# DIG-Beihang/RobustART

Hardware: AMD Instinct MI355X
Metric: corrupted+attacked images/sec/node (ResNet-50, PGD-7 + IN-C x5) (higher is better)
Workload: dtype bf16x3; 1 GPU; per step and GPU: gaussian_noise sev 1..5 on 256 u8 224x224 images -> normalise -> ResNet-50 eval (1280 img) + PGD-Linf-7 eps 2/255 ResNet-50 eval (256 img); global_batch=256, parallelism=dp1, streams=2

## Files before the change

### include/robustart_hip.h

```cpp
#ifndef ROBUSTART_HIP_H
#define ROBUSTART_HIP_H

#include <stddef.h>
#include <stdint.h>

#ifdef __cplusplus
extern "C" {
#endif

typedef void* rart_stream_t;

typedef enum rart_status {
  RART_OK = 0,
  RART_ERR_INVALID = 1,
  RART_ERR_UNSUPPORTED = 2,
  RART_ERR_WORKSPACE = 3,
  RART_ERR_HIP = 4
} rart_status;

enum {
  RART_GAUSSIAN_NOISE = 0, RART_SHOT_NOISE = 1, RART_IMPULSE_NOISE = 2, RART_DEFOCUS_BLUR = 3,
  RART_GLASS_BLUR = 4, RART_MOTION_BLUR = 5, RART_ZOOM_BLUR = 6, RART_SNOW = 7, RART_FROST = 8,
  RART_FOG = 9, RART_BRIGHTNESS = 10, RART_CONTRAST = 11, RART_ELASTIC_TRANSFORM = 12,
  RART_PIXELATE = 13, RART_JPEG_COMPRESSION = 14, RART_SPECKLE_NOISE = 15, RART_GAUSSIAN_BLUR = 16,
// ... 186 lines not shown
typedef struct rart_gemm_pair_cls_desc {
  rart_gemm_pair2_desc two;
  int n_classes, reserved_;
  rart_gemm_pair_class cls[4];
} rart_gemm_pair_cls_desc;
int rart_gemm_pair_classes_bf16(const rart_gemm_pair_cls_desc* desc_host, rart_stream_t stream);
int rart_gemm_pair_max_classes(void);
int rart_gemm_pair_set_schedule(int mode);
int rart_gemm_pair_get_schedule(void);

typedef struct rart_conv_tail_desc {
  const void* a_hi;  const void* a_lo;
  const void* w_hi;  const void* w_lo;
  const void* t_hi;  const void* t_lo;
  const float* bias_mid;
  const float* bias_out;
  const void* mask_mid;  const void* mask_out;
  void* sign_mid;  void* sign_out;
  const void* res_hi;  const void* res_lo;
  void* dst_hi;  void* dst_lo;
  int batch, h, w, c_mid, ldw, relu_mid, relu_out;
  int tap_dy[9], tap_dx[9];
  const void* n_hi;  const void* n_lo;
  const float* bias_next;
  const void* mask_next;
  void* sign_next;
  void* dstn_hi;  void* dstn_lo;
  int relu_next;
  const void* x_hi;  const void* x_lo;
  const void* tx_hi;  const void* tx_lo;
} rart_conv_tail_desc;
int rart_conv3x3_tail_pair_supported(int c_mid);
int rart_conv3x3_tail_pair(const rart_conv_tail_desc* desc_host, rart_stream_t stream);

int rart_vit_add_pos_cls_pair(void* x_hi, void* x_lo, const float* cls_pos0, const float* pos, int n, int tokens, int dim,
                              rart_stream_t stream);
int rart_layernorm_pair(const void* x_hi, const void* x_lo, const float* gamma, const float* beta, void* out_hi, void* out_lo, int rows,
                        int dim, int64_t in_row_stride, int64_t out_row_stride, float eps, rart_stream_t stream);
int rart_layernorm_bwd_pair(const void* dy_hi, const void* dy_lo, const void* x_hi, const void* x_lo, const float* gamma,
                            const void* res_hi, const void* res_lo, void* dx_hi, void* dx_lo, int rows, int dim, int64_t dy_row_stride,
                            int64_t x_row_stride, int64_t res_row_stride, int64_t dx_row_stride, float eps, rart_stream_t stream);
int rart_softmax_rows_pair(const float* scores, void* probs_hi, void* probs_lo, int64_t rows, int n_valid, int ld_in, int ld_out,
                           float scale, rart_stream_t stream);
int rart_softmax_bwd_rows_pair(const void* probs_hi, const void* probs_lo, const float* dprobs, void* ds_hi, void* ds_lo, int64_t rows,
                               int n_valid, int ld_p, int ld_dp, int ld_out, float scale, rart_stream_t stream);
int rart_vit_unpatchify_from_f32(const float* dpatches, float* grad, int n, int h, int w, int patch, int64_t ld, const float* std_host,
                                 rart_stream_t stream);
int rart_vit_attention_pair(const void* qkv_hi, const void* qkv_lo, void* out_hi, void* out_lo, int n, int tokens, int heads, int head_dim,
                            rart_stream_t stream);
int rart_vit_attention_bwd_pair(const void* qkv_hi, const void* qkv_lo, const void* out_hi, const void* out_lo, const void* dout_hi,
                                const void* dout_lo, void* dqkv_hi, void* dqkv_lo, float* stats, int n, int tokens, int heads, int head_dim,
                                rart_stream_t stream);

int rart_conv3x3_halo_supported(int channels, int h, int w);
int rart_conv3x3_pack_frag_bf16(const void* w_rows, void* w_frag, int channels, rart_stream_t stream);
int rart_pack_frag_bf16(const void* w_rows, void* w_frag, int rows, int k, rart_stream_t stream);
int rart_conv3x3_halo_bf16(const void* src, const void* wgt, const float* bias, const void* mask_bits, void* sign_out,
                           void* dst, int n, int h, int w, int channels, const int* tap_dy, const int* tap_dx, int relu,
                           rart_stream_t stream);

int rart_bottleneck_fused_supported(int c_io, int c_mid, int h, int w);
int rart_bottleneck_fused_bf16(const void* x, const void* w1, const void* w2, const void* w3, const float* b1, const float* b2,
                               const float* b3, void* m1, void* m2, void* m3, void* out, int n, int h, int w, int c_io,
                               int c_mid, const int* tap_dy, const int* tap_dx, int backward, rart_stream_t stream);

int rart_bottleneck_first_supported(int c_in, int c_mid, int c_out, int h, int w);
// ... 306 lines not shown
```

### robustart_amd/_lib.py

```python
import ctypes
import os

_HERE = os.path.dirname(os.path.abspath(__file__))
LIB_PATH = os.path.join(_HERE, 'lib', 'librobustart_hip.so')

c_void_p, c_int, c_size_t, c_u64, c_float = (ctypes.c_void_p, ctypes.c_int, ctypes.c_size_t,
                                              ctypes.c_uint64, ctypes.c_float)
c_double = ctypes.c_double

ABI_VERSION = 110

SIGNATURES = {
    'rart_version': (c_int, []),
    'rart_last_error_string': (ctypes.c_char_p, []),
    'rart_corruption_name': (ctypes.c_char_p, [c_int]),
    'rart_corrupt_workspace_bytes': (c_size_t, [c_int, c_int, c_int, c_int, c_int]),
    'rart_corrupt_u8': (c_int, [c_void_p, c_void_p, c_int, c_int, c_int, c_int, c_int, c_u64, c_u64,
                                ctypes.POINTER(c_void_p), c_int, c_void_p, c_size_t, c_void_p]),
    'rart_stencil_fixed_point_info': (c_int, [c_int, c_int, c_void_p, c_void_p, c_size_t]),
    'rart_noise_multi_u8': (c_int, [c_void_p, ctypes.POINTER(c_void_p), c_int, c_int, c_int, c_int, c_int, ctypes.POINTER(c_int),
                                    ctypes.POINTER(c_u64), c_u64, c_void_p]),
    'rart_frost_textures_u8': (c_int, [c_void_p, c_void_p, c_int, c_int, c_int, c_int, c_void_p, c_int, c_int, c_int, ctypes.POINTER(c_int),
                                       c_u64, c_u64, c_void_p]),
    'rart_pil_resize_workspace_bytes': (c_size_t, [c_int] * 10),
# ... 77 lines not shown
    'rart_bottleneck_fused_bf16': (c_int, [c_void_p] * 11 + [c_int] * 5 + [ctypes.POINTER(c_int), ctypes.POINTER(c_int), c_int,
                                           c_void_p]),
    'rart_igemm_set_bk64_min_k': (c_int, [ctypes.c_longlong]),
    'rart_gemm_small_m_bf16': (c_int, [c_void_p, c_int, c_void_p, c_int, c_void_p, c_void_p, c_int, c_int, c_int, c_int, c_int, c_void_p]),
    'rart_igemm_set_gemm256': (c_int, [c_int]),
    'rart_gemm256_supported': (c_int, [ctypes.c_longlong, c_int, c_int, c_int, c_int]),
    'rart_gemm_pair_bf16': (c_int, [c_void_p, c_void_p]),
    'rart_copy_calibration': (c_int, [c_void_p, c_void_p, ctypes.c_size_t, c_int, c_void_p]),
    'rart_gemm_pair_set_schedule': (c_int, [c_int]),
    'rart_gemm_pair_get_schedule': (c_int, []),
    'rart_pack_jobs_bf16': (c_int, [c_void_p, c_int, c_int, c_void_p]),
    'rart_vit_add_pos_cls_pair': (c_int, [c_void_p, c_void_p, c_void_p, c_void_p, c_int, c_int, c_int, c_void_p]),
    'rart_layernorm_pair': (c_int, [c_void_p] * 6 + [c_int, c_int, ctypes.c_int64, ctypes.c_int64, c_float, c_void_p]),
    'rart_layernorm_bwd_pair': (c_int, [c_void_p] * 9 + [c_int, c_int] + [ctypes.c_int64] * 4 + [c_float, c_void_p]),
    'rart_softmax_rows_pair': (c_int, [c_void_p, c_void_p, c_void_p, ctypes.c_int64, c_int, c_int, c_int, c_float, c_void_p]),
    'rart_softmax_bwd_rows_pair': (c_int, [c_void_p] * 5 + [ctypes.c_int64, c_int, c_int, c_int, c_int, c_float, c_void_p]),
    'rart_vit_attention_pair': (c_int, [c_void_p, c_void_p, c_void_p, c_void_p, c_int, c_int, c_int, c_int, c_void_p]),
    'rart_vit_attention_bwd_pair': (c_int, [c_void_p] * 9 + [c_int, c_int, c_int, c_int, c_void_p]),
    'rart_vit_unpatchify_from_f32': (c_int, [c_void_p, c_void_p, c_int, c_int, c_int, c_int, ctypes.c_int64, ctypes.POINTER(c_float), c_void_p]),
    'rart_engine_prep_input': (c_int, [c_void_p, c_int, c_void_p, c_void_p, c_int, c_int, c_int, c_void_p, c_void_p,
                                       c_void_p]),
    'rart_engine_maxpool': (c_int, [c_void_p, c_void_p, c_void_p, c_int, c_int, c_int, c_int, c_void_p]),
    'rart_engine_maxpool_keep': (c_int, [c_void_p, c_void_p, c_void_p, c_void_p, c_int, c_int, c_int, c_int, c_void_p]),
    'rart_engine_maxpool_bwd': (c_int, [c_void_p, c_void_p, c_void_p, c_void_p, c_int, c_int, c_int, c_int, c_void_p]),
    'rart_engine_avgpool': (c_int, [c_void_p, c_void_p, c_int, c_int, c_int, c_void_p]),
    'rart_engine_avgpool_bwd': (c_int, [c_void_p, c_void_p, c_void_p, c_int, c_int, c_int, c_void_p]),
    'rart_engine_stem_col2im': (c_int, [c_void_p, c_void_p, c_int, c_int, c_int, c_int, c_void_p, c_void_p]),
    'rart_engine_stem_fwd_fused': (c_int, [c_void_p, c_int, c_void_p, c_int, c_void_p, c_void_p, c_void_p, c_void_p, c_int, c_int,
                                           c_int, c_void_p, c_void_p, c_void_p]),
    'rart_wgrad_direct_supported': (c_int, [c_int, c_int, c_int]),
    'rart_wgrad_direct_bf16': (c_int, [c_void_p, c_void_p, c_void_p] + [c_int] * 10 + [c_void_p, c_void_p, c_int, c_int, c_int, c_void_p]),
    'rart_conv3x3_tail_pair_supported': (c_int, [c_int]),
    'rart_conv3x3_tail_pair': (c_int, [c_void_p, c_void_p]),
    'rart_engine_stem_fwd_fused_pair': (c_int, [c_void_p, c_int] + [c_void_p] * 7 + [c_int, c_int, c_int, c_void_p, c_void_p, c_void_p]),
    'rart_engine_stem_fwd_next_pair': (c_int, [c_void_p, c_int] + [c_void_p] * 9 + [c_int] + [c_void_p] * 4 + [c_int, c_int, c_int, c_void_p, c_void_p,
                                               c_void_p]),
    'rart_engine_stem_bwd_fused_pair': (c_int, [c_void_p] * 6 + [c_int, c_int, c_int, c_void_p, c_void_p]),
    'rart_engine_stem_bwd_fused': (c_int, [c_void_p, c_void_p, c_void_p, c_void_p, c_int, c_int, c_int, c_void_p, c_void_p]),
    'rart_engine_maxpool_pair': (c_int, [c_void_p, ctypes.c_longlong, c_void_p, ctypes.c_longlong, c_void_p, c_void_p, c_int, c_int, c_int, c_int, c_void_p]),
    'rart_engine_maxpool_bwd_pair': (c_int, [c_void_p, c_void_p, ctypes.c_longlong, c_void_p, ctypes.c_longlong, c_int, c_int, c_int, c_int, c_void_p]),
    'rart_engine_avgpool_pair': (c_int, [c_void_p, ctypes.c_longlong, c_void_p, ctypes.c_longlong, c_int, c_int, c_int, c_void_p]),
    'rart_engine_avgpool_bwd_pair': (c_int, [c_void_p, c_void_p, ctypes.c_longlong, c_void_p, ctypes.c_longlong, c_int, c_int, c_int, c_void_p]),
    'rart_f32_to_pair_rows': (c_int, [c_void_p, c_void_p, ctypes.c_longlong, c_int, c_int, c_int, c_void_p]),
    'rart_engine_stem_col2im_f32': (c_int, [c_void_p, c_void_p, c_int, c_int, c_int, c_int, c_void_p, c_void_p]),
    'rart_f32_to_bf16_rows': (c_int, [c_void_p, c_void_p, c_int, c_int, c_int, c_void_p]),
    'rart_cnx_dwconv_ln_bf16': (c_int, [c_void_p] * 7 + [c_int] * 4 + [c_float, c_void_p]),
    'rart_cnx_dwconv_ln_pair': (c_int, [c_void_p] * 10 + [c_int] * 4 + [c_float, c_void_p]),
    'rart_cnx_dwconv_bwd_bf16': (c_int, [c_void_p] * 4 + [c_int] * 4 + [c_void_p]),
    'rart_cnx_dwconv_bwd_pair': (c_int, [c_void_p] * 7 + [c_int] * 4 + [c_void_p]),
    'rart_cnx_pool_bwd_bf16': (c_int, [c_void_p, c_void_p, c_int, c_int, c_int, c_void_p]),
    'rart_cnx_pool_bwd_pair': (c_int, [c_void_p] * 4 + [c_int, c_int, c_int, c_void_p]),
    'rart_cnx_patchify': (c_int, [c_void_p, c_int, c_void_p, c_void_p, c_int, c_int, c_int, c_int, c_int, c_void_p, c_void_p, c_void_p]),
    'rart_cvst_im2col': (c_int, [c_void_p, c_int, c_void_p, c_void_p, c_int, c_int, c_int, c_int, c_void_p, c_void_p, c_void_p]),
    'rart_cvst_col2im_f32': (c_int, [c_void_p, c_void_p, c_int, c_int, c_int, c_int, c_void_p, c_void_p]),
    'rart_ln_gelu_bf16': (c_int, [c_void_p] * 4 + [c_int, c_int, ctypes.c_int64, ctypes.c_int64, c_float, c_void_p]),
    'rart_ln_gelu_pair': (c_int, [c_void_p] * 6 + [c_int, c_int, ctypes.c_int64, ctypes.c_int64, c_float, c_void_p]),
    'rart_ln_gelu_bwd_bf16': (c_int, [c_void_p] * 5 + [c_int, c_int] + [ctypes.c_int64] * 3 + [c_float, c_void_p]),
    'rart_ln_gelu_bwd_pair': (c_int, [c_void_p] * 8 + [c_int, c_int] + [ctypes.c_int64] * 3 + [c_float, c_void_p]),
    'rart_cnx_dwconv_wgrad_workspace_bytes': (c_size_t, [c_int] * 4),
    'rart_cnx_dwconv_wgrad_bf16': (c_int, [c_void_p] * 4 + [c_int] * 6 + [c_void_p, c_size_t, c_void_p]),
    'rart_cnx_layer_scale_fwd_bf16': (c_int, [c_void_p] * 4 + [ctypes.c_longlong, c_int, c_void_p]),
    'rart_cnx_layer_scale_bwd_workspace_bytes': (c_size_t, [ctypes.c_longlong, c_int]),
    'rart_cnx_layer_scale_bwd_bf16': (c_int, [c_void_p] * 6 + [ctypes.c_longlong, c_int, c_int, c_void_p, c_size_t, c_void_p]),
    'rart_cnx_grn_stats_bf16': (c_int, [c_void_p] * 2 + [c_int] * 3 + [c_void_p]),
    'rart_cnx_grn_stats_pair': (c_int, [c_void_p] * 3 + [c_int] * 3 + [c_void_p]),
    'rart_cnx_grn_apply_bf16': (c_int, [c_void_p] * 5 + [c_int] * 3 + [c_float, c_void_p]),
# ... 260 lines not shown
```

### robustart_amd/csrc/conv_tail_pair.hip

```cpp
#include "rart_common.h"
#include "rart_lds_dma.h"

typedef __attribute__((ext_vector_type(8))) __bf16 bf16x8;
typedef __attribute__((ext_vector_type(16))) float f32x16;

namespace {
constexpr int CT_TM = 128;
constexpr int CT_LDE = 68;
constexpr int CT_PLANE_A = CT_TM * 64;
constexpr int CT_NLD = 144;
constexpr int CT_WREG = 2 * 32 * CT_NLD;
static_assert(CT_WREG >= 32 * CT_LDE * 4, "the staging must fit the wave's region");

struct ConvTailDev {
  const uint16_t *a_hi, *a_lo, *w_hi, *w_lo, *t_hi, *t_lo;
  const float *bias_mid, *bias_out;
  const uint8_t *mask_mid, *mask_out;
  uint8_t *sign_mid, *sign_out;
  const uint16_t *res_hi, *res_lo;
  uint16_t *dst_hi, *dst_lo;
  int M, H, W, ldw, relu_mid, relu_out;
  int tap_dy[9], tap_dx[9];
  uint32_t w_magic, w_shift, h_magic, h_shift;
  const uint16_t *n_hi, *n_lo;
  const float* bias_next;
  const uint8_t* mask_next;
  uint8_t* sign_next;
  uint16_t *dstn_hi, *dstn_lo;
  int relu_next;
  const uint16_t *x_hi, *x_lo, *tx_hi, *tx_lo;
};
typedef __attribute__((ext_vector_type(4))) uint32_t ct_u4;
__device__ __forceinline__ uint4 ct_nt_load(const uint16_t* p) {
  const ct_u4 v = __builtin_nontemporal_load(reinterpret_cast<const ct_u4*>(p));
  return make_uint4(v[0], v[1], v[2], v[3]);
}
__device__ __forceinline__ void ct_nt_store(uint16_t* p, const uint4& v) {
  ct_u4 w = {v.x, v.y, v.z, v.w};
  __builtin_nontemporal_store(w, reinterpret_cast<ct_u4*>(p));
}
__device__ __forceinline__ uint32_t ct_fastdiv(uint32_t n, uint32_t magic, uint32_t shift) { return (uint32_t)(((uint64_t)n * magic) >> shift); }

__device__ __forceinline__ uint32_t ct_pack_bf16x2(float lo, float hi) {
  typedef __attribute__((ext_vector_type(2))) float f2_t;
  typedef __attribute__((ext_vector_type(2))) __bf16 b2_t;
// ... 31 lines not shown

template <int NJ>
__device__ __forceinline__ void ct_pointwise_frags(const f32x16* acc, const uint32_t* mw, bool relu, int h, uint4* fh, uint4* fl) {
#pragma unroll
  for (int j = 0; j < NJ; ++j)
#pragma unroll
    for (int ge = 0; ge < 4; ge += 2) {
      uint32_t eh[2], el[2], oh[2], ol[2];
#pragma unroll
      for (int w = 0; w < 2; ++w) {
        float ve[2], vo[2];
#pragma unroll
        for (int i = 0; i < 2; ++i) {
          ve[i] = acc[j][4 * ge + 2 * w + i];
          vo[i] = acc[j][4 * ge + 4 + 2 * w + i];
          if (relu) { ve[i] = fmaxf(ve[i], 0.f); vo[i] = fmaxf(vo[i], 0.f); }
          if (!((mw[j] >> (8 * ge + 4 * h + 2 * w + i)) & 1u)) ve[i] = 0.f;
          if (!((mw[j] >> (8 * ge + 8 + 4 * h + 2 * w + i)) & 1u)) vo[i] = 0.f;
        }
        eh[w] = ct_pack_bf16x2(ve[0], ve[1]);
        el[w] = ct_pack_bf16x2(ve[0] - __uint_as_float(eh[w] << 16), ve[1] - __uint_as_float(eh[w] & 0xFFFF0000u));
        oh[w] = ct_pack_bf16x2(vo[0], vo[1]);
        ol[w] = ct_pack_bf16x2(vo[0] - __uint_as_float(oh[w] << 16), vo[1] - __uint_as_float(oh[w] & 0xFFFF0000u));
        const auto sh = __builtin_amdgcn_permlane32_swap(eh[w], oh[w], false, false);
        eh[w] = sh[0]; oh[w] = sh[1];
        const auto sl = __builtin_amdgcn_permlane32_swap(el[w], ol[w], false, false);
        el[w] = sl[0]; ol[w] = sl[1];
      }
      fh[j * 2 + ge / 2] = make_uint4(eh[0], eh[1], oh[0], oh[1]);
      fl[j * 2 + ge / 2] = make_uint4(el[0], el[1], ol[0], ol[1]);
    }
}

template <int C, bool NEXT, bool XS = false>
__global__ __launch_bounds__(256, (C == 64 && !NEXT && !XS) ? 3 : 2) void k_conv3x3_tail_pair(const ConvTailDev d) {
  static_assert(!XS || C == 64, "the shortcut source is built for layer1's first block: 64 input channels");
  constexpr int KX = 4;
  constexpr int NJ = C / 32;
  constexpr int KS = C / 16;
  constexpr int NOUT = 4 * C, NC = NOUT / 64;
  constexpr int TPT_SHIFT = C == 64 ? 1 : 2;
  constexpr int KT = 9 << TPT_SHIFT;
  constexpr int PLANE_B = C * 64, STAGE = 2 * CT_PLANE_A + 2 * PLANE_B;
  constexpr int BQ = (C / 16) / 4;
  static_assert(4 * CT_WREG <= 2 * STAGE, "the waves' epilogue regions must fit the tile buffers");
  __shared__ __attribute__((aligned(16))) uint8_t lds[2 * STAGE];
  const int tid = threadIdx.x, lane = tid & 63;
  const int wave = __builtin_amdgcn_readfirstlane(tid >> 6);
  uint32_t tile;
  {
    const uint32_t nb = gridDim.x, bid = blockIdx.x, xcd = bid & 7u, slot = bid >> 3, q = nb >> 3, r = nb & 7u;
    tile = (xcd < r ? xcd * (q + 1u) : r * (q + 1u) + (xcd - r) * q) + slot;
  }
  const int m0 = (int)tile * CT_TM;

  uint32_t avoff[2], nok[2] = {0u, 0u};
  int tap_min = 0;
  for (int t = 0; t < 9; ++t) tap_min = min(tap_min, (d.tap_dy[t] * d.W + d.tap_dx[t]) * (C * 2));
  const int tapreg = lane < 9 ? (d.tap_dy[lane] * d.W + d.tap_dx[lane]) * (C * 2) - tap_min : 0;
#pragma unroll
  for (int q = 0; q < 2; ++q) {
    const int r = 16 * (wave + 4 * q) + (lane >> 2);
    const int cs = ((lane & 3) ^ ((r >> 2) & 3)) * 16;
    const int m = m0 + r;
    const bool ok = m < d.M;
    const uint32_t mm = ok ? (uint32_t)m : 0u;
    const uint32_t t = ct_fastdiv(mm, d.w_magic, d.w_shift);
    const int ax = (int)(mm - t * (uint32_t)d.W);
    const int n = (int)ct_fastdiv(t, d.h_magic, d.h_shift);
    const int ay = (int)(t - (uint32_t)n * (uint32_t)d.H);
    avoff[q] = (uint32_t)((n * d.H * d.W + ay * d.W + ax) * (C * 2) + cs);
    for (int t2 = 0; t2 < 9; ++t2) {
      const int iy = ay + d.tap_dy[t2], ix = ax + d.tap_dx[t2];
      if (!(ok && (unsigned)iy < (unsigned)d.H && (unsigned)ix < (unsigned)d.W)) nok[q] |= 1u << t2;
    }
  }
  uint32_t wvoff[BQ];
#pragma unroll
  for (int q = 0; q < BQ; ++q) {
    const int r = 16 * (wave + 4 * q) + (lane >> 2);
    wvoff[q] = (uint32_t)((r * d.ldw + (((lane & 3) ^ ((r >> 2) & 3)) * 8)) * 2);
  }
  const rart_srd_t srd_ah = rart_dma_srd(reinterpret_cast<const char*>(d.a_hi) + tap_min), srd_al = rart_dma_srd(reinterpret_cast<const char*>(d.a_lo) + tap_min);
  const rart_srd_t srd_wh = rart_dma_srd(d.w_hi), srd_wl = rart_dma_srd(d.w_lo);
  const uint32_t lds_base = (uint32_t)(uintptr_t)(__attribute__((address_space(3))) uint8_t*)lds;
#define RART_CT_ISSUE(KT_, BUF)                                                                                 \
  {                                                                                                             \
    const uint32_t st_ = lds_base + (BUF)*STAGE;                                                                \
    const int kt_ = (KT_);                                                                                      \
    const int tap_ = kt_ >> TPT_SHIFT;                                                                          \
    const uint32_t so_ = (uint32_t)(__builtin_amdgcn_readlane(tapreg, tap_) + (kt_ - (tap_ << TPT_SHIFT)) * 64); \
    _Pragma("unroll") for (int q = 0; q < 2; ++q) {                                                             \
      const uint32_t vo_ = avoff[q] | ((uint32_t)__builtin_amdgcn_sbfe(nok[q], tap_, 1) & RART_DMA_OOR);        \
      rart_dma_load16(vo_, srd_ah, so_, st_ + (wave + 4 * q) * 1024);                                           \
      rart_dma_load16(vo_, srd_al, so_, st_ + CT_PLANE_A + (wave + 4 * q) * 1024);                              \
    }                                                                                                           \
    _Pragma("unroll") for (int q = 0; q < BQ; ++q) {                                                            \
      rart_dma_load16(wvoff[q], srd_wh, (uint32_t)kt_ * 64u, st_ + 2 * CT_PLANE_A + (wave + 4 * q) * 1024);     \
      rart_dma_load16(wvoff[q], srd_wl, (uint32_t)kt_ * 64u, st_ + 2 * CT_PLANE_A + PLANE_B + (wave + 4 * q) * 1024); \
    }                                                                                                           \
  }
  const int fr = lane & 31, h = lane >> 5;
  uint32_t xo[2];
#pragma unroll
  for (int ks = 0; ks < 2; ++ks) xo[ks] = (uint32_t)(fr * 64 + (((2 * ks + h) ^ ((fr >> 2) & 3)) << 4));
  f32x16 acc[NJ];
#pragma unroll
  for (int j = 0; j < NJ; ++j)
#pragma unroll
    for (int g = 0; g < 4; ++g) {
      float4 bv = make_float4(0.f, 0.f, 0.f, 0.f);
      if (d.bias_mid) bv = *reinterpret_cast<const float4*>(d.bias_mid + j * 32 + 8 * g + 4 * h);
      acc[j][4 * g] = bv.x; acc[j][4 * g + 1] = bv.y; acc[j][4 * g + 2] = bv.z; acc[j][4 * g + 3] = bv.w;
    }
  RART_CT_ISSUE(0, 0)
  rart_dma_wait<0>();
  __syncthreads();
  for (int kt = 0; kt < KT; ++kt) {
    const int buf = kt & 1;
    if (kt + 1 < KT) RART_CT_ISSUE(kt + 1, buf ^ 1)
    const uint8_t* Pb = lds + buf * STAGE + (wave * 32) * 64;
    const uint8_t* Wb = lds + buf * STAGE + 2 * CT_PLANE_A;
#pragma unroll
    for (int ks = 0; ks < 2; ++ks) {
      const bf16x8 ph = *reinterpret_cast<const bf16x8*>(Pb + xo[ks]);
      const bf16x8 pl = *reinterpret_cast<const bf16x8*>(Pb + CT_PLANE_A + xo[ks]);
#pragma unroll
      for (int j = 0; j < NJ; ++j) {
        const bf16x8 wh = *reinterpret_cast<const bf16x8*>(Wb + j * 32 * 64 + xo[ks]);
        const bf16x8 wl = *reinterpret_cast<const bf16x8*>(Wb + PLANE_B + j * 32 * 64 + xo[ks]);
        acc[j] = __builtin_amdgcn_mfma_f32_32x32x16_bf16(wh, pl, acc[j], 0, 0, 0);
        acc[j] = __builtin_amdgcn_mfma_f32_32x32x16_bf16(wl, ph, acc[j], 0, 0, 0);
        acc[j] = __builtin_amdgcn_mfma_f32_32x32x16_bf16(wh, ph, acc[j], 0, 0, 0);
      }
    }
    rart_dma_wait<0>();
    __syncthreads();
  }
#undef RART_CT_ISSUE

  const int p = m0 + wave * 32 + fr;
  const bool p_ok = p < d.M;
  bf16x8 a2h[KS], a2l[KS];
  {
    uint32_t mw[NJ];
#pragma unroll
    for (int j = 0; j < NJ; ++j) mw[j] = 0xFFFFFFFFu;
    if (d.mask_mid && p_ok) {
      const uint32_t* mp = reinterpret_cast<const uint32_t*>(d.mask_mid + (size_t)p * (C / 8));
#pragma unroll
      for (int j = 0; j < NJ; ++j) mw[j] = mp[j];
    }
    uint4 fh[KS], fl[KS];
    ct_pointwise_frags<NJ>(acc, mw, d.relu_mid != 0, h, fh, fl);
#pragma unroll
    for (int s = 0; s < KS; ++s) {
      a2h[s] = __builtin_bit_cast(bf16x8, fh[s]);
      a2l[s] = __builtin_bit_cast(bf16x8, fl[s]);
      if (d.sign_mid && p_ok) d.sign_mid[(size_t)p * (C / 8) + 2 * s + h] = (uint8_t)ct_sign_byte(fh[s]);
    }
  }

  bf16x8 xfh[XS ? KX : 1], xfl[XS ? KX : 1];
  if (XS) {
#pragma unroll
    for (int s = 0; s < KX; ++s) {
      uint4 vh = make_uint4(0, 0, 0, 0), vl = vh;
      if (p_ok) {
        vh = *reinterpret_cast<const uint4*>(d.x_hi + (size_t)p * 64 + 16 * s + 8 * h);
        vl = *reinterpret_cast<const uint4*>(d.x_lo + (size_t)p * 64 + 16 * s + 8 * h);
      }
      xfh[s] = __builtin_bit_cast(bf16x8, vh);
// ... 159 lines not shown
      }
      __builtin_amdgcn_fence(__ATOMIC_RELEASE, "wavefront");
      __builtin_amdgcn_wave_barrier();
    }
  }
  if (NEXT) {
    uint32_t mw[NJ];
#pragma unroll
    for (int j = 0; j < NJ; ++j) mw[j] = 0xFFFFFFFFu;
    if (d.mask_next && p_ok) {
      const uint32_t* mp = reinterpret_cast<const uint32_t*>(d.mask_next + (size_t)p * (C / 8));
#pragma unroll
      for (int j = 0; j < NJ; ++j) mw[j] = mp[j];
    }
    uint4 fh[KS], fl[KS];
    ct_pointwise_frags<NJ>(accn, mw, d.relu_next != 0, h, fh, fl);
    if (p_ok) {
#pragma unroll
      for (int s = 0; s < KS; ++s) {
        ct_nt_store(d.dstn_hi + (size_t)p * C + 16 * s + 8 * h, fh[s]);
        ct_nt_store(d.dstn_lo + (size_t)p * C + 16 * s + 8 * h, fl[s]);
        if (d.sign_next) d.sign_next[(size_t)p * (C / 8) + 2 * s + h] = (uint8_t)ct_sign_byte(fh[s]);
      }
    }
  }
}

void ct_magic(uint32_t dv, uint32_t& mg, uint32_t& sh) {
  uint32_t l = 0;
  while ((1ull << l) < dv) ++l;
  sh = 31 + l;
  mg = (uint32_t)(((1ull << sh) + dv - 1) / dv);
}
}

extern "C" int rart_conv3x3_tail_pair_supported(int c_mid) { return (c_mid == 64 || c_mid == 128) ? 1 : 0; }

extern "C" int rart_conv3x3_tail_pair(const rart_conv_tail_desc* t, rart_stream_t stream) {
  RART_CHECK_ARG(t != nullptr, "rart_conv3x3_tail_pair: null descriptor");
  RART_CHECK_ARG(t->a_hi && t->a_lo && t->w_hi && t->w_lo && t->t_hi && t->t_lo && t->dst_hi && t->dst_lo,
                 "rart_conv3x3_tail_pair: null operand plane");
  RART_CHECK_ARG(t->c_mid == 64 || t->c_mid == 128, "rart_conv3x3_tail_pair: c_mid must be 64 or 128 (layer1 / layer2)");
  RART_CHECK_ARG(t->batch > 0 && t->h > 0 && t->w > 0, "rart_conv3x3_tail_pair: empty geometry");
  RART_CHECK_ARG((t->res_hi == nullptr) == (t->res_lo == nullptr), "rart_conv3x3_tail_pair: the skip is a pair: both planes or none");
  RART_CHECK_ARG(t->ldw % 8 == 0 && t->ldw >= 9 * t->c_mid, "rart_conv3x3_tail_pair: ldw must cover 9 taps x c_mid and keep 16-byte alignment");
  const long long M = (long long)t->batch * t->h * t->w;
  RART_CHECK_ARG(M * 4 * t->c_mid < (1ll << 31), "rart_conv3x3_tail_pair: tensors must stay below 2^31 elements (split the batch)");
  const bool xs = t->x_hi != nullptr;
  RART_CHECK_ARG(!xs || (t->x_lo && t->tx_hi && t->tx_lo), "rart_conv3x3_tail_pair: the shortcut source needs both input planes and both table planes");
  RART_CHECK_ARG(!xs || (t->c_mid == 64 && !t->res_hi), "rart_conv3x3_tail_pair: the shortcut source is served at c_mid = 64 and takes the place of the skip pair");
  ConvTailDev d{};
  d.x_hi = (const uint16_t*)t->x_hi; d.x_lo = (const uint16_t*)t->x_lo; d.tx_hi = (const uint16_t*)t->tx_hi; d.tx_lo = (const uint16_t*)t->tx_lo;
  d.a_hi = (const uint16_t*)t->a_hi; d.a_lo = (const uint16_t*)t->a_lo; d.w_hi = (const uint16_t*)t->w_hi; d.w_lo = (const uint16_t*)t->w_lo;
  d.t_hi = (const uint16_t*)t->t_hi; d.t_lo = (const uint16_t*)t->t_lo;
  d.bias_mid = t->bias_mid; d.bias_out = t->bias_out;
  d.mask_mid = (const uint8_t*)t->mask_mid; d.mask_out = (const uint8_t*)t->mask_out;
  d.sign_mid = (uint8_t*)t->sign_mid; d.sign_out = (uint8_t*)t->sign_out;
  d.res_hi = (const uint16_t*)t->res_hi; d.res_lo = (const uint16_t*)t->res_lo;
  d.dst_hi = (uint16_t*)t->dst_hi; d.dst_lo = (uint16_t*)t->dst_lo;
  d.M = (int)M; d.H = t->h; d.W = t->w; d.ldw = t->ldw; d.relu_mid = t->relu_mid; d.relu_out = t->relu_out;
  for (int i = 0; i < 9; ++i) { d.tap_dy[i] = t->tap_dy[i]; d.tap_dx[i] = t->tap_dx[i]; }
  const bool next = t->n_hi != nullptr;
  RART_CHECK_ARG(!next || (t->n_lo && t->dstn_hi && t->dstn_lo), "rart_conv3x3_tail_pair: the neighbour's reduction needs both table planes and its destination pair");
  d.n_hi = (const uint16_t*)t->n_hi; d.n_lo = (const uint16_t*)t->n_lo; d.bias_next = t->bias_next; d.mask_next = (const uint8_t*)t->mask_next;
  d.sign_next = (uint8_t*)t->sign_next; d.dstn_hi = (uint16_t*)t->dstn_hi; d.dstn_lo = (uint16_t*)t->dstn_lo; d.relu_next = t->relu_next;
  ct_magic((uint32_t)d.W, d.w_magic, d.w_shift);
  ct_magic((uint32_t)d.H, d.h_magic, d.h_shift);
  const dim3 grid((uint32_t)((M + CT_TM - 1) / CT_TM));
  hipStream_t st = (hipStream_t)stream;
  if (xs) {
    if (next) hipLaunchKernelGGL((k_conv3x3_tail_pair<64, true, true>), grid, dim3(256), 0, st, d);
    else hipLaunchKernelGGL((k_conv3x3_tail_pair<64, false, true>), grid, dim3(256), 0, st, d);
  } else if (t->c_mid == 64) {
    if (next) hipLaunchKernelGGL((k_conv3x3_tail_pair<64, true>), grid, dim3(256), 0, st, d);
    else hipLaunchKernelGGL((k_conv3x3_tail_pair<64, false>), grid, dim3(256), 0, st, d);
  } else {
    if (next) hipLaunchKernelGGL((k_conv3x3_tail_pair<128, true>), grid, dim3(256), 0, st, d);
    else hipLaunchKernelGGL((k_conv3x3_tail_pair<128, false>), grid, dim3(256), 0, st, d);
  }
  RART_CHECK_LAUNCH("rart_conv3x3_tail_pair");
  return RART_OK;
}
```

Measured before the change: 8975 images/s.

## Stage conv3x3 tail input as a halo slab once per tile instead of per tap

```diff
diff --git a/include/robustart_hip.h b/include/robustart_hip.h
--- a/include/robustart_hip.h
+++ b/include/robustart_hip.h
@@ -242,6 +242,8 @@
 } rart_conv_tail_desc;
 int rart_conv3x3_tail_pair_supported(int c_mid);
 int rart_conv3x3_tail_pair(const rart_conv_tail_desc* desc_host, rart_stream_t stream);
+int rart_conv3x3_tail_pair_set_staging(int mode);
+int rart_conv3x3_tail_pair_get_staging(void);
 
 int rart_vit_add_pos_cls_pair(void* x_hi, void* x_lo, const float* cls_pos0, const float* pos, int n, int tokens, int dim,
                               rart_stream_t stream);
diff --git a/robustart_amd/_lib.py b/robustart_amd/_lib.py
--- a/robustart_amd/_lib.py
+++ b/robustart_amd/_lib.py
@@ -133,6 +133,8 @@
     'rart_wgrad_direct_bf16': (c_int, [c_void_p, c_void_p, c_void_p] + [c_int] * 10 + [c_void_p, c_void_p, c_int, c_int, c_int, c_void_p]),
     'rart_conv3x3_tail_pair_supported': (c_int, [c_int]),
     'rart_conv3x3_tail_pair': (c_int, [c_void_p, c_void_p]),
+    'rart_conv3x3_tail_pair_set_staging': (c_int, [c_int]),
+    'rart_conv3x3_tail_pair_get_staging': (c_int, []),
     'rart_engine_stem_fwd_fused_pair': (c_int, [c_void_p, c_int] + [c_void_p] * 7 + [c_int, c_int, c_int, c_void_p, c_void_p, c_void_p]),
     'rart_engine_stem_fwd_next_pair': (c_int, [c_void_p, c_int] + [c_void_p] * 9 + [c_int] + [c_void_p] * 4 + [c_int, c_int, c_int, c_void_p, c_void_p,
                                                c_void_p]),
diff --git a/robustart_amd/csrc/conv_tail_pair.hip b/robustart_amd/csrc/conv_tail_pair.hip
--- a/robustart_amd/csrc/conv_tail_pair.hip
+++ b/robustart_amd/csrc/conv_tail_pair.hip
@@ -11,6 +11,8 @@
 constexpr int CT_NLD = 144;
 constexpr int CT_WREG = 2 * 32 * CT_NLD;
 static_assert(CT_WREG >= 32 * CT_LDE * 4, "the staging must fit the wave's region");
+constexpr int CT_SLAB_ROWS = 248;
+constexpr int CT_SLAB_IMG = CT_SLAB_ROWS * 64;
 
 struct ConvTailDev {
   const uint16_t *a_hi, *a_lo, *w_hi, *w_lo, *t_hi, *t_lo;
@@ -108,9 +110,10 @@
     }
 }
 
-template <int C, bool NEXT, bool XS = false>
-__global__ __launch_bounds__(256, (C == 64 && !NEXT && !XS) ? 3 : 2) void k_conv3x3_tail_pair(const ConvTailDev d) {
+template <int C, bool NEXT, bool XS = false, bool SLAB = false>
+__global__ __launch_bounds__(256, (C == 64 && !NEXT && !XS && !SLAB) ? 3 : 2) void k_conv3x3_tail_pair(const ConvTailDev d) {
   static_assert(!XS || C == 64, "the shortcut source is built for layer1's first block: 64 input channels");
+  static_assert(!SLAB || C == 64, "the slab is sized for 64 channels (124 KB at 128)");
   constexpr int KX = 4;
   constexpr int NJ = C / 32;
   constexpr int KS = C / 16;
@@ -119,8 +122,10 @@
   constexpr int KT = 9 << TPT_SHIFT;
   constexpr int PLANE_B = C * 64, STAGE = 2 * CT_PLANE_A + 2 * PLANE_B;
   constexpr int BQ = (C / 16) / 4;
-  static_assert(4 * CT_WREG <= 2 * STAGE, "the waves' epilogue regions must fit the tile buffers");
-  __shared__ __attribute__((aligned(16))) uint8_t lds[2 * STAGE];
+  constexpr int SLAB_W = 4 * CT_SLAB_IMG;
+  constexpr int LDS_BYTES = SLAB ? SLAB_W + 4 * PLANE_B : 2 * STAGE;
+  static_assert(4 * CT_WREG <= (SLAB ? SLAB_W : 2 * STAGE), "the waves' epilogue regions must fit the tile buffers");
+  __shared__ __attribute__((aligned(16))) uint8_t lds[LDS_BYTES];
   const int tid = threadIdx.x, lane = tid & 63;
   const int wave = __builtin_amdgcn_readfirstlane(tid >> 6);
   uint32_t tile;
@@ -129,53 +134,6 @@
     tile = (xcd < r ? xcd * (q + 1u) : r * (q + 1u) + (xcd - r) * q) + slot;
   }
   const int m0 = (int)tile * CT_TM;
-
-  uint32_t avoff[2], nok[2] = {0u, 0u};
-  int tap_min = 0;
-  for (int t = 0; t < 9; ++t) tap_min = min(tap_min, (d.tap_dy[t] * d.W + d.tap_dx[t]) * (C * 2));
-  const int tapreg = lane < 9 ? (d.tap_dy[lane] * d.W + d.tap_dx[lane]) * (C * 2) - tap_min : 0;
-#pragma unroll
-  for (int q = 0; q < 2; ++q) {
-    const int r = 16 * (wave + 4 * q) + (lane >> 2);
-    const int cs = ((lane & 3) ^ ((r >> 2) & 3)) * 16;
-    const int m = m0 + r;
-    const bool ok = m < d.M;
-    const uint32_t mm = ok ? (uint32_t)m : 0u;
-    const uint32_t t = ct_fastdiv(mm, d.w_magic, d.w_shift);
-    const int ax = (int)(mm - t * (uint32_t)d.W);
-    const int n = (int)ct_fastdiv(t, d.h_magic, d.h_shift);
-    const int ay = (int)(t - (uint32_t)n * (uint32_t)d.H);
-    avoff[q] = (uint32_t)((n * d.H * d.W + ay * d.W + ax) * (C * 2) + cs);
-    for (int t2 = 0; t2 < 9; ++t2) {
-      const int iy = ay + d.tap_dy[t2], ix = ax + d.tap_dx[t2];
-      if (!(ok && (unsigned)iy < (unsigned)d.H && (unsigned)ix < (unsigned)d.W)) nok[q] |= 1u << t2;
-    }
-  }
-  uint32_t wvoff[BQ];
-#pragma unroll
-  for (int q = 0; q < BQ; ++q) {
-    const int r = 16 * (wave + 4 * q) + (lane >> 2);
-    wvoff[q] = (uint32_t)((r * d.ldw + (((lane & 3) ^ ((r >> 2) & 3)) * 8)) * 2);
-  }
-  const rart_srd_t srd_ah = rart_dma_srd(reinterpret_cast<const char*>(d.a_hi) + tap_min), srd_al = rart_dma_srd(reinterpret_cast<const char*>(d.a_lo) + tap_min);
-  const rart_srd_t srd_wh = rart_dma_srd(d.w_hi), srd_wl = rart_dma_srd(d.w_lo);
-  const uint32_t lds_base = (uint32_t)(uintptr_t)(__attribute__((address_space(3))) uint8_t*)lds;
-#define RART_CT_ISSUE(KT_, BUF)                                                                                 \
-  {                                                                                                             \
-    const uint32_t st_ = lds_base + (BUF)*STAGE;                                                                \
-    const int kt_ = (KT_);                                                                                      \
-    const int tap_ = kt_ >> TPT_SHIFT;                                                                          \
-    const uint32_t so_ = (uint32_t)(__builtin_amdgcn_readlane(tapreg, tap_) + (kt_ - (tap_ << TPT_SHIFT)) * 64); \
-    _Pragma("unroll") for (int q = 0; q < 2; ++q) {                                                             \
-      const uint32_t vo_ = avoff[q] | ((uint32_t)__builtin_amdgcn_sbfe(nok[q], tap_, 1) & RART_DMA_OOR);        \
-      rart_dma_load16(vo_, srd_ah, so_, st_ + (wave + 4 * q) * 1024);                                           \
-      rart_dma_load16(vo_, srd_al, so_, st_ + CT_PLANE_A + (wave + 4 * q) * 1024);                              \
-    }                                                                                                           \
-    _Pragma("unroll") for (int q = 0; q < BQ; ++q) {                                                            \
-      rart_dma_load16(wvoff[q], srd_wh, (uint32_t)kt_ * 64u, st_ + 2 * CT_PLANE_A + (wave + 4 * q) * 1024);     \
-      rart_dma_load16(wvoff[q], srd_wl, (uint32_t)kt_ * 64u, st_ + 2 * CT_PLANE_A + PLANE_B + (wave + 4 * q) * 1024); \
-    }                                                                                                           \
-  }
   const int fr = lane & 31, h = lane >> 5;
   uint32_t xo[2];
 #pragma unroll
@@ -189,31 +147,161 @@
       if (d.bias_mid) bv = *reinterpret_cast<const float4*>(d.bias_mid + j * 32 + 8 * g + 4 * h);
       acc[j][4 * g] = bv.x; acc[j][4 * g + 1] = bv.y; acc[j][4 * g + 2] = bv.z; acc[j][4 * g + 3] = bv.w;
     }
-  RART_CT_ISSUE(0, 0)
-  rart_dma_wait<0>();
-  __syncthreads();
-  for (int kt = 0; kt < KT; ++kt) {
-    const int buf = kt & 1;
-    if (kt + 1 < KT) RART_CT_ISSUE(kt + 1, buf ^ 1)
-    const uint8_t* Pb = lds + buf * STAGE + (wave * 32) * 64;
-    const uint8_t* Wb = lds + buf * STAGE + 2 * CT_PLANE_A;
-#pragma unroll
-    for (int ks = 0; ks < 2; ++ks) {
-      const bf16x8 ph = *reinterpret_cast<const bf16x8*>(Pb + xo[ks]);
-      const bf16x8 pl = *reinterpret_cast<const bf16x8*>(Pb + CT_PLANE_A + xo[ks]);
-#pragma unroll
-      for (int j = 0; j < NJ; ++j) {
-        const bf16x8 wh = *reinterpret_cast<const bf16x8*>(Wb + j * 32 * 64 + xo[ks]);
-        const bf16x8 wl = *reinterpret_cast<const bf16x8*>(Wb + PLANE_B + j * 32 * 64 + xo[ks]);
-        acc[j] = __builtin_amdgcn_mfma_f32_32x32x16_bf16(wh, pl, acc[j], 0, 0, 0);
-        acc[j] = __builtin_amdgcn_mfma_f32_32x32x16_bf16(wl, ph, acc[j], 0, 0, 0);
-        acc[j] = __builtin_amdgcn_mfma_f32_32x32x16_bf16(wh, ph, acc[j], 0, 0, 0);
-      }
-    }
+
+  if constexpr (SLAB) {
+    rart_srd_t srd_ah = rart_dma_srd(d.a_hi), srd_al = rart_dma_srd(d.a_lo);
+    srd_ah[2] = srd_al[2] = (uint32_t)d.M * (uint32_t)(C * 2);
+    const rart_srd_t srd_wh = rart_dma_srd(d.w_hi), srd_wl = rart_dma_srd(d.w_lo);
+    const uint32_t lds_base = (uint32_t)(uintptr_t)(__attribute__((address_space(3))) uint8_t*)lds;
+    const int halo = d.W + 1;
+    const uint32_t lane_off = (uint32_t)((((lane & 3) ^ ((lane >> 4) & 3)) << 4));
+#pragma unroll
+    for (int q = 0; q < 4; ++q) {
+      const int piece = wave + 4 * q;
+      const int srow = 16 * piece + (lane >> 2);
+      const int pos = m0 - halo + srow;
+      const uint32_t vo = (uint32_t)pos < (uint32_t)d.M ? (uint32_t)pos * (uint32_t)(C * 2) + lane_off : RART_DMA_OOR;
+      if (srow < CT_SLAB_ROWS) {
+#pragma unroll
+        for (int kh = 0; kh < 2; ++kh) {
+          rart_dma_load16(vo + kh * 64, srd_ah, 0u, lds_base + (2 * kh) * CT_SLAB_IMG + piece * 1024);
+          rart_dma_load16(vo + kh * 64, srd_al, 0u, lds_base + (2 * kh + 1) * CT_SLAB_IMG + piece * 1024);
+        }
+      }
+    }
+    const int wr = 16 * wave + (lane >> 2);
+    const uint32_t wvoff = (uint32_t)((wr * d.ldw + (((lane & 3) ^ ((wr >> 2) & 3)) * 8)) * 2);
+#define RART_CT_ISSUE_W(KT_, BUF)                                                              \
+  {                                                                                            \
+    const uint32_t st_ = lds_base + SLAB_W + (BUF) * 2 * PLANE_B + wave * 1024;                \
+    rart_dma_load16(wvoff, srd_wh, (uint32_t)(KT_) * 64u, st_);                                \
+    rart_dma_load16(wvoff, srd_wl, (uint32_t)(KT_) * 64u, st_ + PLANE_B);                      \
+  }
+    RART_CT_ISSUE_W(0, 0)
+    uint32_t nokf = 0u;
+    {
+      const int m = m0 + wave * 32 + fr;
+      const bool ok = m < d.M;
+      const uint32_t mm = ok ? (uint32_t)m : 0u;
+      const uint32_t t = ct_fastdiv(mm, d.w_magic, d.w_shift);
+      const int ax = (int)(mm - t * (uint32_t)d.W);
+      const int ay = (int)(t - ct_fastdiv(t, d.h_magic, d.h_shift) * (uint32_t)d.H);
+      for (int t2 = 0; t2 < 9; ++t2) {
+        const int iy = ay + d.tap_dy[t2], ix = ax + d.tap_dx[t2];
+        if (!(ok && (unsigned)iy < (unsigned)d.H && (unsigned)ix < (unsigned)d.W)) nokf |= 1u << t2;
+      }
+    }
+    const int tapreg = lane < 9 ? d.tap_dy[lane] * d.W + d.tap_dx[lane] : 0;
+    const int rbase = wave * 32 + fr + halo;
     rart_dma_wait<0>();
     __syncthreads();
-  }
+#pragma unroll
+    for (int j = 0; j < NJ; ++j) asm volatile("" : "+v"(acc[j]));
+#pragma unroll 1
+    for (int tap = 0; tap < 9; ++tap) {
+      const int R = rbase + __builtin_amdgcn_readlane(tapreg, tap);
+      const bool zero = ((nokf >> tap) & 1u) != 0u;
+      uint32_t so[2];
+#pragma unroll
+      for (int ks = 0; ks < 2; ++ks) so[ks] = (uint32_t)(R * 64 + (((2 * ks + h) ^ ((R >> 2) & 3)) << 4));
+#pragma unroll
+      for (int kh = 0; kh < 2; ++kh) {
+        if (2 * tap + kh + 1 < KT) RART_CT_ISSUE_W(2 * tap + kh + 1, kh ^ 1)
+        const uint8_t* Pb = lds + (2 * kh) * CT_SLAB_IMG;
+        const uint8_t* Wb = lds + SLAB_W + kh * 2 * PLANE_B;
+#pragma unroll
+        for (int ks = 0; ks < 2; ++ks) {
+          uint4 vh = *reinterpret_cast<const uint4*>(Pb + so[ks]);
+          uint4 vl = *reinterpret_cast<const uint4*>(Pb + CT_SLAB_IMG + so[ks]);
+          if (zero) vh = vl = make_uint4(0u, 0u, 0u, 0u);
+          const bf16x8 ph = __builtin_bit_cast(bf16x8, vh), pl = __builtin_bit_cast(bf16x8, vl);
+#pragma unroll
+          for (int j = 0; j < NJ; ++j) {
+            const bf16x8 wh = *reinterpret_cast<const bf16x8*>(Wb + j * 32 * 64 + xo[ks]);
+            const bf16x8 wl = *reinterpret_cast<const bf16x8*>(Wb + PLANE_B + j * 32 * 64 + xo[ks]);
+            acc[j] = __builtin_amdgcn_mfma_f32_32x32x16_bf16(wh, pl, acc[j], 0, 0, 0);
+            acc[j] = __builtin_amdgcn_mfma_f32_32x32x16_bf16(wl, ph, acc[j], 0, 0, 0);
+            acc[j] = __builtin_amdgcn_mfma_f32_32x32x16_bf16(wh, ph, acc[j], 0, 0, 0);
+          }
+        }
+        rart_dma_wait<0>();
+        __syncthreads();
+      }
+    }
+#undef RART_CT_ISSUE_W
+  } else {
+    uint32_t avoff[2], nok[2] = {0u, 0u};
+    int tap_min = 0;
+    for (int t = 0; t < 9; ++t) tap_min = min(tap_min, (d.tap_dy[t] * d.W + d.tap_dx[t]) * (C * 2));
+    const int tapreg = lane < 9 ? (d.tap_dy[lane] * d.W + d.tap_dx[lane]) * (C * 2) - tap_min : 0;
+#pragma unroll
+    for (int q = 0; q < 2; ++q) {
+      const int r = 16 * (wave + 4 * q) + (lane >> 2);
+      const int cs = ((lane & 3) ^ ((r >> 2) & 3)) * 16;
+      const int m = m0 + r;
+      const bool ok = m < d.M;
+      const uint32_t mm = ok ? (uint32_t)m : 0u;
+      const uint32_t t = ct_fastdiv(mm, d.w_magic, d.w_shift);
+      const int ax = (int)(mm - t * (uint32_t)d.W);
+      const int n = (int)ct_fastdiv(t, d.h_magic, d.h_shift);
+      const int ay = (int)(t - (uint32_t)n * (uint32_t)d.H);
+      avoff[q] = (uint32_t)((n * d.H * d.W + ay * d.W + ax) * (C * 2) + cs);
+      for (int t2 = 0; t2 < 9; ++t2) {
+        const int iy = ay + d.tap_dy[t2], ix = ax + d.tap_dx[t2];
+        if (!(ok && (unsigned)iy < (unsigned)d.H && (unsigned)ix < (unsigned)d.W)) nok[q] |= 1u << t2;
+      }
+    }
+    uint32_t wvoff[BQ];
+#pragma unroll
+    for (int q = 0; q < BQ; ++q) {
+      const int r = 16 * (wave + 4 * q) + (lane >> 2);
+      wvoff[q] = (uint32_t)((r * d.ldw + (((lane & 3) ^ ((r >> 2) & 3)) * 8)) * 2);
+    }
+    const rart_srd_t srd_ah = rart_dma_srd(reinterpret_cast<const char*>(d.a_hi) + tap_min), srd_al = rart_dma_srd(reinterpret_cast<const char*>(d.a_lo) + tap_min);
+    const rart_srd_t srd_wh = rart_dma_srd(d.w_hi), srd_wl = rart_dma_srd(d.w_lo);
+    const uint32_t lds_base = (uint32_t)(uintptr_t)(__attribute__((address_space(3))) uint8_t*)lds;
+#define RART_CT_ISSUE(KT_, BUF)                                                                                 \
+    {                                                                                                             \
+      const uint32_t st_ = lds_base + (BUF)*STAGE;                                                                \
+      const int kt_ = (KT_);                                                                                      \
+      const int tap_ = kt_ >> TPT_SHIFT;                                                                          \
+      const uint32_t so_ = (uint32_t)(__builtin_amdgcn_readlane(tapreg, tap_) + (kt_ - (tap_ << TPT_SHIFT)) * 64); \
+      _Pragma("unroll") for (int q = 0; q < 2; ++q) {                                                             \
+        const uint32_t vo_ = avoff[q] | ((uint32_t)__builtin_amdgcn_sbfe(nok[q], tap_, 1) & RART_DMA_OOR);        \
+        rart_dma_load16(vo_, srd_ah, so_, st_ + (wave + 4 * q) * 1024);                                           \
+        rart_dma_load16(vo_, srd_al, so_, st_ + CT_PLANE_A + (wave + 4 * q) * 1024);                              \
+      }                                                                                                           \
+      _Pragma("unroll") for (int q = 0; q < BQ; ++q) {                                                            \
+        rart_dma_load16(wvoff[q], srd_wh, (uint32_t)kt_ * 64u, st_ + 2 * CT_PLANE_A + (wave + 4 * q) * 1024);     \
+        rart_dma_load16(wvoff[q], srd_wl, (uint32_t)kt_ * 64u, st_ + 2 * CT_PLANE_A + PLANE_B + (wave + 4 * q) * 1024); \
+      }                                                                                                           \
+    }
+    RART_CT_ISSUE(0, 0)
+    rart_dma_wait<0>();
+    __syncthreads();
+    for (int kt = 0; kt < KT; ++kt) {
+      const int buf = kt & 1;
+      if (kt + 1 < KT) RART_CT_ISSUE(kt + 1, buf ^ 1)
+      const uint8_t* Pb = lds + buf * STAGE + (wave * 32) * 64;
+      const uint8_t* Wb = lds + buf * STAGE + 2 * CT_PLANE_A;
+#pragma unroll
+      for (int ks = 0; ks < 2; ++ks) {
+        const bf16x8 ph = *reinterpret_cast<const bf16x8*>(Pb + xo[ks]);
+        const bf16x8 pl = *reinterpret_cast<const bf16x8*>(Pb + CT_PLANE_A + xo[ks]);
+#pragma unroll
+        for (int j = 0; j < NJ; ++j) {
+          const bf16x8 wh = *reinterpret_cast<const bf16x8*>(Wb + j * 32 * 64 + xo[ks]);
+          const bf16x8 wl = *reinterpret_cast<const bf16x8*>(Wb + PLANE_B + j * 32 * 64 + xo[ks]);
+          acc[j] = __builtin_amdgcn_mfma_f32_32x32x16_bf16(wh, pl, acc[j], 0, 0, 0);
+          acc[j] = __builtin_amdgcn_mfma_f32_32x32x16_bf16(wl, ph, acc[j], 0, 0, 0);
+          acc[j] = __builtin_amdgcn_mfma_f32_32x32x16_bf16(wh, ph, acc[j], 0, 0, 0);
+        }
+      }
+      rart_dma_wait<0>();
+      __syncthreads();
+    }
 #undef RART_CT_ISSUE
+  }
 
   const int p = m0 + wave * 32 + fr;
   const bool p_ok = p < d.M;
@@ -439,7 +527,23 @@
   sh = 31 + l;
   mg = (uint32_t)(((1ull << sh) + dv - 1) / dv);
 }
-}
+
+int g_tail_staging = -1;
+int ct_staging() {
+  if (g_tail_staging < 0) {
+    const char* e = getenv("RART_TAIL_STAGING");
+    g_tail_staging = (e && atoi(e) == 0) ? 0 : 1;
+  }
+  return g_tail_staging;
+}
+}
+
+extern "C" int rart_conv3x3_tail_pair_set_staging(int mode) {
+  RART_CHECK_ARG(mode == 0 || mode == 1, "rart_conv3x3_tail_pair_set_staging: mode must be 0 (input staged per tap) or 1 (input slab staged once per tile)");
+  g_tail_staging = mode;
+  return RART_OK;
+}
+extern "C" int rart_conv3x3_tail_pair_get_staging(void) { return ct_staging(); }
 
 extern "C" int rart_conv3x3_tail_pair_supported(int c_mid) { return (c_mid == 64 || c_mid == 128) ? 1 : 0; }
 
@@ -475,7 +579,17 @@
   ct_magic((uint32_t)d.H, d.h_magic, d.h_shift);
   const dim3 grid((uint32_t)((M + CT_TM - 1) / CT_TM));
   hipStream_t st = (hipStream_t)stream;
-  if (xs) {
+  bool slab = ct_staging() == 1 && t->c_mid == 64 && CT_TM + 2 * (t->w + 1) <= CT_SLAB_ROWS;
+  for (int i = 0; i < 9; ++i) slab = slab && t->tap_dy[i] >= -1 && t->tap_dy[i] <= 1 && t->tap_dx[i] >= -1 && t->tap_dx[i] <= 1;
+  if (slab) {
+    if (xs) {
+      if (next) hipLaunchKernelGGL((k_conv3x3_tail_pair<64, true, true, true>), grid, dim3(256), 0, st, d);
+      else hipLaunchKernelGGL((k_conv3x3_tail_pair<64, false, true, true>), grid, dim3(256), 0, st, d);
+    } else {
+      if (next) hipLaunchKernelGGL((k_conv3x3_tail_pair<64, true, false, true>), grid, dim3(256), 0, st, d);
+      else hipLaunchKernelGGL((k_conv3x3_tail_pair<64, false, false, true>), grid, dim3(256), 0, st, d);
+    }
+  } else if (xs) {
     if (next) hipLaunchKernelGGL((k_conv3x3_tail_pair<64, true, true>), grid, dim3(256), 0, st, d);
     else hipLaunchKernelGGL((k_conv3x3_tail_pair<64, false, true>), grid, dim3(256), 0, st, d);
   } else if (t->c_mid == 64) {
diff --git a/scratch/time_tail_staging.py b/scratch/time_tail_staging.py
--- /dev/null
+++ b/scratch/time_tail_staging.py
@@ -0,0 +1,80 @@
+import ctypes, sys, os, json
+sys.path.insert(0, os.path.dirname(os.path.dirname(os.path.abspath(__file__))))
+import torch
+from robustart_amd import _lib
+
+lib = _lib.load()
+sp = _lib.stream_ptr
+B = int(sys.argv[1]) if len(sys.argv) > 1 else 256
+H = W = 56
+C, N = 64, 256
+P = B * H * W
+
+
+def pairt(*shape):
+    return (torch.randn(2, *shape, device='cuda') * 0.5).to(torch.bfloat16)
+
+
+def timeit(d, reps=10, groups=3):
+    for _ in range(3):
+        _lib.check(lib.rart_conv3x3_tail_pair(ctypes.byref(d), sp()))
+    torch.cuda.synchronize()
+    ts = []
+    for _ in range(groups):
+        a, b = torch.cuda.Event(enable_timing=True), torch.cuda.Event(enable_timing=True)
+        a.record()
+        for _ in range(reps):
+            _lib.check(lib.rart_conv3x3_tail_pair(ctypes.byref(d), sp()))
+        b.record()
+        torch.cuda.synchronize()
+        ts.append(round(a.elapsed_time(b) / reps * 1000, 1))
+    return sorted(ts)
+
+
+src, dst, res, dstn, x = pairt(P, C), pairt(P, N), pairt(P, N), pairt(P, C), pairt(P, C)
+tab = (torch.randn(C, 3 * 9 * C, device='cuda') * 0.05).to(torch.bfloat16)
+tail, ntab, tx = pairt(N * C) * 0.1, pairt(N * C) * 0.1, pairt(N * C) * 0.1
+b2, b3, bn = torch.randn(C, device='cuda'), torch.randn(N, device='cuda'), torch.randn(C, device='cuda')
+sm, so, sn = (torch.zeros(P, c // 8, dtype=torch.uint8, device='cuda') for c in (C, N, C))
+mm, mo, mn = (torch.randint(0, 256, (P, c // 8), dtype=torch.uint8, device='cuda') for c in (C, N, C))
+
+
+def desc(nxt, xs, backward):
+    d = _lib.ConvTailDesc()
+    d.a_hi, d.a_lo, d.w_hi, d.w_lo = src[0].data_ptr(), src[1].data_ptr(), tab.data_ptr(), tab.data_ptr() + 2 * 9 * C
+    d.t_hi, d.t_lo, d.dst_hi, d.dst_lo = tail[0].data_ptr(), tail[1].data_ptr(), dst[0].data_ptr(), dst[1].data_ptr()
+    d.batch, d.h, d.w, d.c_mid, d.ldw = B, H, W, C, 3 * 9 * C
+    for i in range(9):
+        d.tap_dy[i], d.tap_dx[i] = (1 - i // 3, 1 - i % 3) if backward else (i // 3 - 1, i % 3 - 1)
+    if xs:
+        d.x_hi, d.x_lo, d.tx_hi, d.tx_lo = x[0].data_ptr(), x[1].data_ptr(), tx[0].data_ptr(), tx[1].data_ptr()
+    else:
+        d.res_hi, d.res_lo = res[0].data_ptr(), res[1].data_ptr()
+    if backward:
+        d.mask_mid, d.mask_out = mm.data_ptr(), mo.data_ptr()
+    else:
+        d.bias_mid, d.bias_out, d.sign_mid, d.sign_out = b2.data_ptr(), b3.data_ptr(), sm.data_ptr(), so.data_ptr()
+        d.relu_mid = d.relu_out = 1
+    if nxt:
+        d.n_hi, d.n_lo, d.dstn_hi, d.dstn_lo = ntab[0].data_ptr(), ntab[1].data_ptr(), dstn[0].data_ptr(), dstn[1].data_ptr()
+        if backward:
+            d.mask_next = mn.data_ptr()
+        else:
+            d.bias_next, d.sign_next, d.relu_next = bn.data_ptr(), sn.data_ptr(), 1
+    return d
+
+
+old = lib.rart_conv3x3_tail_pair_get_staging()
+try:
+    for name, nxt, xs, backward in (('next_fwd', 1, 0, 0), ('next_bwd', 1, 0, 1), ('next_xs_fwd', 1, 1, 0), ('plain_fwd', 0, 0, 0), ('plain_bwd', 0, 0, 1)):
+        d = desc(nxt, xs, backward)
+        r, outs = {}, {}
+        for staging in (0, 1, 0, 1):
+            _lib.check(lib.rart_conv3x3_tail_pair_set_staging(staging))
+            key = ('per_tap', 'slab')[staging] + ('_again' if ('per_tap', 'slab')[staging] in r else '')
+            r[key] = timeit(d)
+            outs[staging] = (dst.view(torch.int16).clone(), dstn.view(torch.int16).clone())
+        r['bit_identical'] = bool(torch.equal(outs[0][0], outs[1][0]) and (not nxt or torch.equal(outs[0][1], outs[1][1])))
+        print(name, json.dumps(r), flush=True)
+finally:
+    lib.rart_conv3x3_tail_pair_set_staging(old)
```

Result: faster. 9112 images/s, median of 6 (+1.5%).
